# lasgroup/safe-adaptation-gym

Measured on AMD Instinct MI355X. Metric: env-steps/sec (batched) Point/GoToGoal, higher is better.
Workload: dtype f32

## Files before the change

safe_adaptation_gym_amd/csrc/sag_device.hpp:

```cpp
#pragma once
#include <hip/hip_runtime.h>
#include <stdint.h>

#include <type_traits>

#include "../../include/sag.h"

namespace sag {

constexpr int WAVE = 64;

enum { DI_META = 0, DI_TSTATE = 1, DI_STEP = 2, DI_ENVID = 3, DI_FLAGS = 4, DI_COUNT = 5 };
constexpr int FLAG_EPISODE_SHIFT = 8;
__host__ __device__ constexpr size_t ipad(size_t N) { return (N + 3) & ~(size_t)3; }
__host__ __device__ constexpr size_t icount(size_t N) { return ipad(N) + 4 * N; }
__host__ __device__ constexpr size_t iaddr(int w, size_t N, size_t i) {
  return w == DI_TSTATE ? i : ipad(N) + i * 4 + (w == DI_META ? 0 : (w == DI_STEP ? 1 : (w == DI_ENVID ? 2 : 3)));
}

constexpr int DEV_FLOATS = 192, DEV_GROUPS = DEV_FLOATS / 4;
constexpr int DV_POS = 40, DV_VEL = 76, DG_HAZ = 5, DG_POS = 10, DG_PILLARS = 4, DG_BUTTONS = 28;
__host__ __device__ constexpr int didx(int k) {
  return k < 6 ? k
       : k < 9 ? 136 + (k - 6)
       : k < 12 ? k
       : k < 14 ? k
       : k < 24 ? 140 + (k - 14)
       : k == 24 ? 38
       : k < 27 ? 14 + (k - 25)
       : k < 32 ? 130 + (k - 27)
       : k < 34 ? 6 + (k - 32)
       : k < 38 ? 124 + (k - 34)
       : k == 38 ? 8
       : k < 41 ? 128 + (k - 39)
       : k < 44 ? DV_POS + 30 + (k - 41)
       : k < 47 ? DV_VEL + 30 + (k - 44)
       : k < 65 ? 20 + (k - 47)
       : k < 69 ? 16 + (k - 65)
       : k < 81 ? 112 + (k - 69)
       : k < 141 ? ((k - 81) % 6 < 3 ? DV_POS + 3 * ((k - 81) / 6) + (k - 81) % 6
                                     : DV_VEL + 3 * ((k - 81) / 6) + (k - 81) % 6 - 3)
       : k == 141 ? 39
       : k < 144 ? 150 + (k - 142)
       : 152 + (k - 144);
}
static_assert(didx(SAG_F_BUTTONS) == 112 && didx(SAG_F_VASES + 6 * 3 + 4) == DV_VEL + 10 && didx(SAG_F_BOX + 1) == DV_POS + 31 &&
              didx(SAG_F_HAZARDS) == 4 * DG_HAZ && didx(SAG_F_PILLARS) == 4 * DG_PILLARS, "device layout constants");
__host__ __device__ constexpr size_t saddr(int k, size_t N, size_t i) {
  return ((size_t)(didx(k) >> 2) * N + i) * 4 + (didx(k) & 3);
}

__host__ __device__ inline uint32_t pack_meta(const int32_t* ri) {
  return (uint32_t)ri[SAG_I_TASK] | (uint32_t)ri[SAG_I_NH] << 4 | (uint32_t)ri[SAG_I_NV] << 8 |
         (uint32_t)ri[SAG_I_NP] << 12 | (uint32_t)ri[SAG_I_NB] << 14 |
         (uint32_t)ri[SAG_I_BOX_KIND] << 17;
}
__host__ __device__ inline void unpack_meta(uint32_t m, int32_t* ri) {
  ri[SAG_I_TASK] = m & 15; ri[SAG_I_NH] = m >> 4 & 15; ri[SAG_I_NV] = m >> 8 & 15;
  ri[SAG_I_NP] = m >> 12 & 3; ri[SAG_I_NB] = m >> 14 & 7; ri[SAG_I_BOX_KIND] = m >> 17 & 3;
}
__host__ __device__ inline uint32_t pack_tstate(const int32_t* ri) {
  return (uint32_t)ri[SAG_I_GOAL_BUTTON] | (uint32_t)ri[SAG_I_BTN_STATE] << 3 |
         (uint32_t)ri[SAG_I_BTN_TIMER] << 4 | (uint32_t)ri[SAG_I_CATCH_TIMER] << 7 |
         (uint32_t)ri[SAG_I_ACTIVE_MASK] << 11;
}
__host__ __device__ inline void unpack_tstate(uint32_t t, int32_t* ri) {
  ri[SAG_I_GOAL_BUTTON] = t & 7; ri[SAG_I_BTN_STATE] = t >> 3 & 1; ri[SAG_I_BTN_TIMER] = t >> 4 & 7;
  ri[SAG_I_CATCH_TIMER] = t >> 7 & 15; ri[SAG_I_ACTIVE_MASK] = t >> 11 & 63;
}

// ... 755 lines not shown
  auto G4 = [&](int g) { return S4[(size_t)g * N + i]; };
  const bool use_hot = MODE == MODE_BUSY && p.hot != nullptr;
  const float4* __restrict__ H4 = use_hot ? reinterpret_cast<const float4*>(p.hot) + (size_t)i * HOT_GROUPS : nullptr;
  auto GH = [&](int g, int hslot) { return use_hot ? H4[hslot] : G4(g); };
  int4 iw;
  uint32_t tstate;
  if (use_hot) {
    const float4 hi = H4[14], ht = H4[15];
    iw = make_int4(__float_as_int(hi.x), __float_as_int(hi.y), __float_as_int(hi.z), __float_as_int(hi.w));
    tstate = (uint32_t)__float_as_int(ht.x);
  } else {
    iw = reinterpret_cast<const int4*>(I + ipad((size_t)N))[i];
    tstate = (uint32_t)I[iaddr(DI_TSTATE, (size_t)N, (size_t)i)];
  }
  const uint32_t meta = (uint32_t)iw.x;
  int step = iw.y;
  const uint32_t env_id = (uint32_t)iw.z;
  const float4 gA = GH(0, 0), gB = GH(1, 1), gC = GH(2, 2), gD = GH(3, 3);
  BV R;
  R.x = gA.x; R.y = gA.y;
  float yaw = gA.z;
  R.vx = gA.w; R.vy = gB.x; R.w = gB.y;
  R.ax = R.ay = R.aw = 0; R.dyn = 1;
  const float gear = gC.y, damp = gC.z;
  const float vsz = gD.z, psz = gD.w;
  float ext[9] = {0, 0, 0, 0, 0, 1, 0, 0, 0}, eacc[5] = {0, 0, 0, 0, 0};
  constexpr int DG_EXT = (152 >> 2);
  static_assert(didx(SAG_F_ROBOT_EXT) == 152 && didx(SAG_F_ROBOT_EXT + 8) == 160, "car extension = device groups 38..40");
  float4 ext_tail = make_float4(0.f, 0.f, 0.f, 0.f);
  if constexpr (CAR) {
    const float4 e0 = G4(DG_EXT), e1 = G4(DG_EXT + 1);
    ext_tail = G4(DG_EXT + 2);
    ext[0] = e0.x; ext[1] = e0.y; ext[2] = e0.z; ext[3] = e0.w; ext[4] = e1.x; ext[5] = e1.y; ext[6] = e1.z; ext[7] = e1.w;
    ext[8] = ext_tail.x;
    if constexpr (PARK) {
      CPK(CP_Q) = ext[5]; CPK(CP_Q + 1) = ext[6]; CPK(CP_Q + 2) = ext[7]; CPK(CP_Q + 3) = ext[8];
      CPK(CP_TAIL) = ext_tail.y; CPK(CP_TAIL + 1) = ext_tail.z; CPK(CP_TAIL + 2) = ext_tail.w;
    }
  }
  float goalx = gB.z, goaly = gB.w;
  float last0 = gC.x;
  float a0 = 0, a1 = 0, n0 = 0, n1 = 0;
  if (!p.observe_only) {
    if constexpr (!DOGGO) {
      const float2 a = reinterpret_cast<const float2*>(p.actions)[i];
      a0 = a.x; a1 = a.y;
      if (p.noise) { const float2 z = reinterpret_cast<const float2*>(p.noise)[i]; n0 = z.x; n1 = z.y; }
    }
  }
  {
    float vpos[36];
    const int need = HAS_TBOX && p.has_box ? 9 : (3 * capV + 3) / 4;
#pragma unroll
    for (int g = 0; g < 9; g++) {
      float4 v = make_float4(0.f, 0.f, 0.f, 0.f);
      if (g < need) v = GH(DG_POS + g, 5 + g);
      vpos[4 * g] = v.x; vpos[4 * g + 1] = v.y; vpos[4 * g + 2] = v.z; vpos[4 * g + 3] = v.w;
    }
#pragma unroll
    for (int k = 0; k < SAG_MAX_VASES; k++)
      if (k >= capV) { vpos[3 * k] = vpos[3 * k + 1] = vpos[3 * k + 2] = 0; }
    if (!(HAS_TBOX && p.has_box)) { vpos[3 * BOX_ID] = vpos[3 * BOX_ID + 1] = vpos[3 * BOX_ID + 2] = 0; }
#pragma unroll
    for (int k = 0; k < NBODY; k++) { LP(LS_X, k) = vpos[3 * k]; LP(LS_Y, k) = vpos[3 * k + 1]; LP(LS_YAW, k) = vpos[3 * k + 2]; }
  }
  float stx[NSTAT], sty[NSTAT];
  {
    float4 v = make_float4(0.f, 0.f, 0.f, 0.f);
    if (capP > 0) v = GH(DG_PILLARS, 4);
    stx[0] = v.x; sty[0] = v.y; stx[1] = capP > 1 ? v.z : 0.f; sty[1] = capP > 1 ? v.w : 0.f;
    static_assert(SAG_MAX_PILLARS == 2, "pillars fill one group");
  }
  if constexpr (HAS_BTN) {
    float bt[12];
#pragma unroll
    for (int g = 0; g < 3; g++) {
      float4 v = make_float4(0.f, 0.f, 0.f, 0.f);
      if (2 * g < capB) v = G4(DG_BUTTONS + g);
      bt[4 * g] = v.x; bt[4 * g + 1] = v.y; bt[4 * g + 2] = v.z; bt[4 * g + 3] = v.w;
    }
    static_assert(SAG_MAX_BUTTONS == 6, "buttons fill three groups");
#pragma unroll
    for (int k = 0; k < SAG_MAX_BUTTONS; k++) {
      stx[SAG_MAX_PILLARS + k] = k < capB ? bt[2 * k] : 0.f;
      sty[SAG_MAX_PILLARS + k] = k < capB ? bt[2 * k + 1] : 0.f;
    }
  }
// ... 15 lines not shown
    if (!p.observe_only) {
      const float an = SF(SAG_F_ACTION_NOISE);
#pragma unroll 1
      for (int j = 0; j < 12; j += 2) {
        float z0, z1;
        if (p.noise) { z0 = p.noise[(size_t)i * 12 + j]; z1 = p.noise[(size_t)i * 12 + j + 1]; }
        else {
          uint32_t c[4] = {rng.env, rng.step, (uint32_t)(j >> 1), rng.ep4 | 1u};
          philox4x32_10(c, p.key0, p.key1);
          box_muller(c[0], c[1], z0, z1);
        }
        const float l0 = SF(SAG_F_CTRL_SCALE + j), l1 = SF(SAG_F_CTRL_SCALE + j + 1);
        ctrl12[j] = clampf(p.actions[(size_t)i * 12 + j] + an * z0, -l0, l0);
        ctrl12[j + 1] = clampf(p.actions[(size_t)i * 12 + j + 1] + an * z1, -l1, l1);
      }
    }
  }
  if (!p.observe_only) {
    if (!p.noise && !DOGGO) {
      uint32_t c[4] = {rng.env, rng.step, 0u, rng.ep4 | 1u};
      philox4x32_10(c, p.key0, p.key1);
      box_muller(c[0], c[1], n0, n1);
    }
    const float an = gC.w;
    const float cs0 = gD.x, cs1 = gD.y;
    ctrl0 = clampf(a0 + an * n0, -cs0, cs0);
    ctrl1 = clampf(a1 + an * n1, -cs1, cs1);
    if (task == SAG_TASK_CATCH_GOAL) {
      int t = tstate >> 7 & 15;
      t = t - 1 > 0 ? t - 1 : 0;
      float cur = SF(SAG_F_CATCH + 2), nxt = SF(SAG_F_CATCH + 3);
      if (t == 0) {
        cur = nxt;
        nxt = (float)rng.uniform(0.2, 1.0);
        if (rng.exhausted) flags |= 2;
        if (live) { SF(SAG_F_CATCH + 2) = cur; SF(SAG_F_CATCH + 3) = nxt; }
        t = 10;
      }
      tstate = (tstate & ~(15u << 7)) | (uint32_t)t << 7;
      double time = (double)step * p.nstep_table * (double)p.h;
      double progress = (10 - t) / 10.0;
      double radius = progress * ((double)nxt - (double)cur) + (double)cur;
      goalx = (float)((double)SF(SAG_F_CATCH) + sin(time) * radius);
      goaly = (float)((double)SF(SAG_F_CATCH + 1) + cos(time) * radius);
    }
  }

  const float h = p.h;
// ... 86 lines not shown
      dgr.cost_contacts = (int)dr[15]; dgr.btn_mask = (uint32_t)dr[16]; dgr.overflow = (int)dr[17];
    } else {
      static_assert(post, "the Doggo physics is k_doggo_physics (sag_doggo_coop.hpp); the generic step only post-processes its results");
    }
    cost_contacts = dgr.cost_contacts; btn_mask = dgr.btn_mask;
    if (dgr.overflow) flags |= 4;
    float wz;
    if (!p.observe_only && live && !post) dg_store(dgs, S, (size_t)N, (size_t)i, yaw, wz);
    else { double Rm[9], ww[3]; dg_quat2mat(dgs.quat, Rm); dg_matvec(Rm, dgs.wloc, ww); yaw = (float)atan2(Rm[3], Rm[0]); wz = (float)ww[2]; }
    {
      double Rm[9];
      dg_quat2mat(dgs.quat, Rm);
      for (int k = 0; k < 9; k++) dg_rot[k] = Rm[k];
    }
    R.x = (float)dgs.pos[0]; R.y = (float)dgs.pos[1]; R.vx = (float)dgs.vlin[0]; R.vy = (float)dgs.vlin[1]; R.w = wz;
    R.ax = (float)dgr.qacc_lin[0]; R.ay = (float)dgr.qacc_lin[1];
    if (nsub > 0) awake = 0;
    for (int k = 0; k < NBODY; k++) {
      const bool isb = k == BOX_ID;
      if (isb ? !has_box : k >= nV) continue;
      LP(LS_X, k) = Wd.fb[k][0]; LP(LS_Y, k) = Wd.fb[k][1]; LP(LS_YAW, k) = Wd.fb[k][2];
      if (Wd.fb[k][3] != 0 || Wd.fb[k][4] != 0 || Wd.fb[k][5] != 0) awake |= 1u << k;
      if (!p.observe_only && live && !post) {
        for (int c = 0; c < 3; c++) { SD(DV_POS + 3 * k + c) = Wd.fb[k][c]; SD(DV_VEL + 3 * k + c) = Wd.fb[k][3 + c]; }
      }
    }
  } else {
  float car_f0 = 0, car_f1 = 0, car_f2 = 0, car_px = 0, car_py = 0, car_pw = 0;
  float car_fL = 0, car_fT = 0, car_fR = 0, car_fX = 0, car_fY = 0;
  bool car_warm = false;
  auto car_floor = [&](const float a0, const float a1, const float a2) {
#pragma clang fp contract(on)
    constexpr float CM = CAR_M, CIO = CAR_IO, COY = CAR_OY, CJD = 0.001f, CRW = 0.05f, AB = -CM * COY;
    constexpr float CNL = CM * GRAV * (0.1f + COY) / 0.4f, CNC = CM * GRAV - 2 * CNL;
    constexpr float IDC = 1.0f / (CM * (CM * CIO - AB * AB));
    constexpr float M0 = (CM * CIO) * IDC, M2 = (-AB * CM) * IDC, M3 = (CM * CIO - AB * AB) * IDC, M5 = (CM * CM) * IDC;
    constexpr float UL0 = -0.13f * M2, UL2 = -0.13f * M5, UT0 = M0 - 0.1f * M2, UT2 = M2 - 0.1f * M5, UX0 = M0 + 0.1f * M2, UX2 = M2 + 0.1f * M5;
    constexpr float LIML = MU * CNL, LIMT = 2 * MU * CNL, LIMC = MU * CNC;
    const float vbx = cy * R.vx + sy * R.vy, vby = cy * R.vy - sy * R.vx, bc = sol0.bcoef;
    const float qL = (clampf(ctrl0, -0.02f, 0.02f) - CJD * ext[0]) * p.car.iIw, qR = (clampf(ctrl1, -0.02f, 0.02f) - CJD * ext[1]) * p.car.iIw;
    const float qX = CJD * ext[3] * p.car.iIb, qY = -CJD * ext[2] * p.car.iIb;
    const float rL = -bc * (vby - 0.13f * R.w + CRW * ext[0]), rT = -bc * (vbx - 0.1f * R.w), rR = -bc * (vby + 0.13f * R.w + CRW * ext[1]);
    const float rX = -bc * (vbx + 0.1f * R.w - CRW * ext[3]), rY = -bc * (vby + CRW * ext[2]);
    const float cL = rL - CRW * qL, cR = rR - CRW * qR, cX = rX - CRW * qX, cY = rY - CRW * qY;
    float fL, fT, fR, fX, fY;
    if constexpr (PARK) { fL = CPK(CP_FL); fT = CPK(CP_FL + 1); fR = CPK(CP_FL + 2); fX = CPK(CP_FL + 3); fY = CPK(CP_FL + 4); }
    else { fL = car_fL; fT = car_fT; fR = car_fR; fX = car_fX; fY = car_fY; }
// ... 332 lines not shown
    ext_tail.y = CPK(CP_TAIL); ext_tail.z = CPK(CP_TAIL + 1); ext_tail.w = CPK(CP_TAIL + 2);
  }

  }
  if (p.ext_cc) {
    const int32_t v = p.ext_cc[i];
    if (v >= 0) { cost_contacts = v; btn_mask = p.ext_btn[i]; }
  }
  CYC(CY_ROBOT);
  const float boxx = LP(LS_X, BOX_ID), boxy = LP(LS_Y, BOX_ID);
  if (!p.observe_only && live) {
    if constexpr (!DOGGO) {
      float4* __restrict__ W4 = reinterpret_cast<float4*>(S);
      W4[(size_t)0 * N + i] = make_float4(R.x, R.y, yaw, R.vx);
    }
    if constexpr (CAR) {
      float4* __restrict__ W4 = reinterpret_cast<float4*>(S);
      W4[(size_t)DG_EXT * N + i] = make_float4(ext[0], ext[1], ext[2], ext[3]);
      W4[(size_t)(DG_EXT + 1) * N + i] = make_float4(ext[4], ext[5], ext[6], ext[7]);
      W4[(size_t)(DG_EXT + 2) * N + i] = make_float4(ext[8], ext_tail.y, ext_tail.z, ext_tail.w);
    }
    for (uint32_t m = dirty; m; m &= m - 1) {
      const int k = __ffs(m) - 1;
      const int f = DV_POS + 3 * k, fv = DV_VEL + 3 * k;
      SD(f) = LP(LS_X, k); SD(f + 1) = LP(LS_Y, k); SD(f + 2) = LP(LS_YAW, k);
      const int d = dy.slot(k);
      if (d >= 0) { SD(fv) = POOL(d, 0); SD(fv + 1) = POOL(d, 1); SD(fv + 2) = POOL(d, 2); }
    }
    step += 1;
    reinterpret_cast<int4*>(I + ipad((size_t)N))[i] = make_int4(iw.x, step, iw.z, iw.w);
  }
  tstate = (tstate & ~(TS_AWAKE_BITS << TS_AWAKE_SHIFT)) | (awake & TS_AWAKE_BITS) << TS_AWAKE_SHIFT;
  bool busy_next = false;
  if (!p.observe_only) {
    const float T = p.nstep_table * h;
    const float amax = CAR ? GRAV : 1.05f * gear * PT_FLIM / PT_MASS;
    const float reach = sqrtf(R.vx * R.vx + R.vy * R.vy) * T + amax * T * T + 0.005f;
    bool busy = awake != 0 || (HAS_TBOX && task == SAG_TASK_HAUL_BOX);
    bool near_obj = false, near_static = false;
    const bool moving = busy;
    const float rr = my_bound + reach;
    constexpr bool FINE = !CAR && !DOGGO;
    const float dth = (fmaxf(fabsf(R.w), 3.0f) + 1.0f) * T;
    const float fa = 0.1f + reach, fb = 0.0707107f + reach + 0.1f * dth;
    const float Bx = R.x + 0.1f * cy, By = R.y + 0.1f * sy;
#pragma unroll 1
    for (int k = 0; k < nV; k++) {
      const float vx_ = LP(LS_X, k), vy_ = LP(LS_Y, k);
      const float dx = vx_ - R.x, dyy = vy_ - R.y, rs = rr + vase_r;
      if (dx * dx + dyy * dyy <= rs * rs) {
        if constexpr (FINE) {
          float sv, cv; sincosf(LP(LS_YAW, k), &sv, &cv);
          auto box_d2 = [&](float px, float py) {
            const float wx = px - vx_, wy = py - vy_;
            const float ex = fmaxf(fabsf(cv * wx + sv * wy) - vsz, 0.f), ey = fmaxf(fabsf(cv * wy - sv * wx) - vsz, 0.f);
            return ex * ex + ey * ey;
          };
          busy |= box_d2(R.x, R.y) <= fa * fa || box_d2(Bx, By) <= fb * fb;
        } else busy = true;
      }
    }
    if (has_box) {
      const float dx = LP(LS_X, BOX_ID) - R.x, dyy = LP(LS_Y, BOX_ID) - R.y, rs = rr + box_r;
      near_obj = dx * dx + dyy * dyy <= rs * rs;
    }
#pragma unroll 1
    for (int k = 0; k < n_static; k++) {
      if (k == capP) k = SAG_MAX_PILLARS;
      const bool is_p = k < SAG_MAX_PILLARS;
      const bool on = is_p ? (k < nP) : (k - SAG_MAX_PILLARS < nB);
      const float sr = is_p ? psz : BUTTON_R;
      const float skx = pick(stx, k), sky = pick(sty, k);
      const float dx = skx - R.x, dyy = sky - R.y, rs = rr + sr;
      if constexpr (FINE) {
        const float ex = skx - Bx, ey = sky - By;
        near_static |= on && (dx * dx + dyy * dyy <= (fa + sr) * (fa + sr) || ex * ex + ey * ey <= (fb + sr) * (fb + sr));
      } else near_static |= on && dx * dx + dyy * dyy <= rs * rs;
    }
    const bool near_vase = busy && !moving;
    busy |= near_obj || near_static;
    const uint32_t kind = p.busy_kinds ? (uint32_t)near_obj | (uint32_t)near_static << 1 | (uint32_t)(near_vase || moving) << 2 : 0u;
    const uint32_t nbit = TS_BUSY_BIT << (p.phase ^ 1);
    tstate = busy ? (tstate | nbit) : (tstate & ~nbit);
    if (busy && live && p.kind) p.kind[i] = (uint8_t)kind;
    busy_next = busy;
  }

  CYC(CY_WRITEBACK);
  float hzx[SAG_MAX_HAZARDS], hzy[SAG_MAX_HAZARDS];
  float hsz;
  {
    float hz[20];
#pragma unroll
    for (int g = 0; g < 5; g++) {
      float4 v = make_float4(0.f, 0.f, 0.f, 0.f);
      if (g == 4 || 2 * g < capH) v = use_hot ? reinterpret_cast<const float4*>(p.hot_haz)[(size_t)i * 5 + g] : G4(DG_HAZ + g);
      hz[4 * g] = v.x; hz[4 * g + 1] = v.y; hz[4 * g + 2] = v.z; hz[4 * g + 3] = v.w;
    }
    static_assert(SAG_MAX_HAZARDS == 9, "hazards + size fill five groups");
#pragma unroll
    for (int k = 0; k < SAG_MAX_HAZARDS; k++) { hzx[k] = k < capH ? hz[2 * k] : 0.f; hzy[k] = k < capH ? hz[2 * k + 1] : 0.f; }
    hsz = hz[18];
  }

  bool bad = false;
  {
    float v[6] = {R.x, R.y, yaw, R.vx, R.vy, R.w};
#pragma unroll
    for (int k = 0; k < 6; k++) bad |= !(fabsf(v[k]) <= 1e10f);
    if constexpr (DOGGO) {
      bad |= !(fabs(dgs.pos[2]) <= 1e10) || !(fabs(dgs.vlin[2]) <= 1e10);
      for (int k = 0; k < 4; k++) bad |= !(fabs(dgs.quat[k]) <= 1e10);
      for (int k = 0; k < 3; k++) bad |= !(fabs(dgs.wloc[k]) <= 1e10);
      for (int k = 0; k < DG_NJ; k++) bad |= !(fabs(dgs.q[k]) <= 1e10) || !(fabs(dgs.qd[k]) <= 1e10);
    }
  }

  double rew0 = 0, rew1 = 0;
  int met = 0;
  const double rx = R.x, ry = R.y;
  bool need_goal = false;
  float box_last1 = 0, box_last2 = 0;
  if (!p.observe_only && !bad) {
    if (task == SAG_TASK_PRESS_BUTTONS || task == SAG_TASK_PRESS_BUTTONS_SCARCE) {
      int gb = tstate & 7, bstate = tstate >> 3 & 1, timer = tstate >> 4 & 7;
// ... 143 lines not shown
    }
  }
  CYC(CY_RESAMPLE);
  if (!p.observe_only && !bad) {
    if (need_goal) {
      last0 = (float)dist2d(rx, ry, goalx, goaly);
      if (task == SAG_TASK_CATCH_GOAL && live) { SF(SAG_F_CATCH) = goalx; SF(SAG_F_CATCH + 1) = goaly; }
      if (has_box) {
        box_last2 = (float)dist2d(goalx, goaly, boxx, boxy);
        box_last1 = (float)dist2d(rx, ry, boxx, boxy);
      }
    }
    if (live) {
      if (has_box) { SF(SAG_F_LAST + 1) = box_last1; SF(SAG_F_LAST + 2) = box_last2; }
      if constexpr (DOGGO) {
        SF(SAG_F_LAST) = last0;
        SF(SAG_F_GOAL) = goalx; SF(SAG_F_GOAL + 1) = goaly;
      }
    }
  }
  if constexpr (!DOGGO) {
    if (!p.observe_only && live) {
      float4* __restrict__ W4 = reinterpret_cast<float4*>(S);
      W4[(size_t)1 * N + i] = make_float4(R.vy, R.w, bad ? gB.z : goalx, bad ? gB.w : goaly);
      W4[(size_t)2 * N + i] = make_float4(bad ? gC.x : last0, gC.y, gC.z, gC.w);
    }
  }
  if (!p.observe_only && live) I[iaddr(DI_TSTATE, (size_t)N, (size_t)i)] = (int32_t)tstate;
  if constexpr (MODE != MODE_ALL && !DOGGO) {
    if (p.hot && busy_next && live && !p.observe_only) {
      float4* __restrict__ Hw = reinterpret_cast<float4*>(p.hot) + (size_t)i * HOT_GROUPS;
      Hw[0] = make_float4(R.x, R.y, yaw, R.vx);
      Hw[1] = make_float4(R.vy, R.w, bad ? gB.z : goalx, bad ? gB.w : goaly);
      Hw[2] = make_float4(bad ? gC.x : last0, gC.y, gC.z, gC.w);
      Hw[3] = gD;
      Hw[4] = make_float4(stx[0], sty[0], stx[1], sty[1]);
#pragma unroll
      for (int g = 0; g < 9; g++) {
        float v[4];
#pragma unroll
        for (int c = 0; c < 4; c++) {
          const int f = 4 * g + c, k = f / 3, comp = f % 3;
          v[c] = k < NBODY ? lds[((comp == 0 ? LS_X : (comp == 1 ? LS_Y : LS_YAW)) + k) * WAVE + lane] : 0.f;
        }
        Hw[5 + g] = make_float4(v[0], v[1], v[2], v[3]);
      }
      Hw[14] = make_float4(__int_as_float(iw.x), __int_as_float(step), __int_as_float(iw.z), __int_as_float(iw.w | flags));
      Hw[15] = make_float4(__int_as_float((int)tstate), 0.f, 0.f, 0.f);
    }
  }

  int cost = 0;
  if (!p.observe_only && !bad) {
    int c = cost_contacts;
#pragma unroll 1
    for (int k = 0; k < SAG_MAX_HAZARDS; k++) {
      if (k < nH) {
        const float dx = R.x - hzx[k], dyy = R.y - hzy[k];
        const float d2 = dx * dx + dyy * dyy, t2 = hsz * hsz;
        bool in = d2 <= t2;
        if (fabsf(d2 - t2) < 1e-5f) in = dist2d(rx, ry, hzx[k], hzy[k]) <= (double)hsz;
        c += in;
      }
    }
    cost = c > 0;
  }
// ... 230 lines not shown
  const bool live = gi < p.N && lane < epw;
  step_body<ROBOT, HAS_BTN, HAS_TBOX, MODE_ALL>(p, lds, lane, live ? gi : p.N - 1, live, base,
                                                 min(epw, p.N - base), 0ull, nullptr);
}

template <bool HAS_BTN, bool HAS_TBOX>
__global__ __launch_bounds__(WAVE, 1) void k_step_doggo_post(StepArgs p) {
  __shared__ float lds[LDS_FLOATS];
  const int lane = threadIdx.x, base = blockIdx.x * WAVE, gi = base + lane;
  const bool live = gi < p.N;
  step_body<SAG_ROBOT_DOGGO, HAS_BTN, HAS_TBOX, MODE_POST>(p, lds, lane, live ? gi : p.N - 1, live, base, min(WAVE, p.N - base),
                                                            0ull, nullptr);
}

#ifndef SAG_QUIET_MIN_WAVES
#define SAG_QUIET_MIN_WAVES 4
#endif
#ifndef SAG_CAR_QUIET_MIN_WAVES
#define SAG_CAR_QUIET_MIN_WAVES 3
#endif
template <int ROBOT, bool HAS_BTN, bool HAS_TBOX>
__global__ __launch_bounds__(WAVE, ROBOT == SAG_ROBOT_CAR ? SAG_CAR_QUIET_MIN_WAVES : SAG_QUIET_MIN_WAVES) void k_step_quiet(StepArgs p) {
  constexpr int QSLOTS = quiet_lds_rows(ROBOT, HAS_BTN, HAS_TBOX);
  static_assert(QSLOTS >= LS_YAW + NBODY, "the yaw rows written at load time must stay in bounds");
  static_assert(QSLOTS * WAVE * (int)sizeof(float) <= quiet_lds_total(ROBOT), "the quiet array stays inside the footprint of its launch");
  __shared__ float lds[QSLOTS * WAVE];
  const int lane = threadIdx.x, base = blockIdx.x * WAVE, gi = base + lane;
  const bool in = gi < p.N;
  const bool busy = in && ((uint32_t)p.I[iaddr(DI_TSTATE, (size_t)p.N, (size_t)gi)] & (TS_BUSY_BIT << p.phase));
  const uint64_t skip = __ballot(busy || !in);
  if (skip == ~0ull) return;
  const bool live = in && !busy;
  step_body<ROBOT, HAS_BTN, HAS_TBOX, MODE_QUIET>(p, lds, lane, in ? gi : p.N - 1, live, base,
                                                   min(WAVE, p.N - base), skip, nullptr);
}

constexpr int COMPACT_PER_LANE = 16, COMPACT_ENVS = 256 * COMPACT_PER_LANE;
template <bool KINDS>
__global__ __launch_bounds__(256) void k_compact(const int32_t* I, const uint8_t* kind, int N, int phase, int32_t* rows, int32_t* count,
                                                  int32_t* zero_for_next, const int32_t* prev_total, int kinds_min) {
  constexpr int NC = KINDS ? BUSY_CLASSES : 1;
  const bool use_kinds = KINDS && *prev_total > kinds_min;
  if (blockIdx.x == 0 && threadIdx.x < BUSY_CLASSES) zero_for_next[threadIdx.x] = 0;
  __shared__ int wave_tot[4][BUSY_CLASSES];
  __shared__ int wave_base[4][BUSY_CLASSES];
  const int lane = threadIdx.x & 63, wv = threadIdx.x >> 6;
  const int e0 = blockIdx.x * COMPACT_ENVS + wv * (WAVE * COMPACT_PER_LANE);
// ... 59 lines not shown
#pragma unroll
  for (int k = 0; k < BUSY_CLASSES; k++) {
    const int c = busy_class_order(k), n = p.count[c], w = (n + WAVE - 1) / WAVE;
    if (cls < 0) { if (b < w) { cls = c; count = n; } else b -= w; }
  }
  if (cls < 0) return;
  const int lane = threadIdx.x, c0 = b * WAVE;
  const int nval = min(WAVE, count - c0);
  const bool live = lane < nval;
  const int i = p.rows[(size_t)cls * p.N + c0 + (live ? lane : 0)];
  rows[lane] = i;
  __syncthreads();
  step_body<ROBOT, HAS_BTN, HAS_TBOX, MODE_BUSY>(p, lds, lane, i, live, 0, nval, 0ull, rows);
#ifdef SAG_WAVE_TIMES
  if (lane == 0 && blockIdx.x < WT_MAX) { g_wt[blockIdx.x][0] = wt0; g_wt[blockIdx.x][1] = wall_clock64(); }
#endif
}

__device__ inline void hot_refresh_env(const float* __restrict__ S, const int32_t* __restrict__ I, int N, size_t i,
                                       float* __restrict__ hot, float* __restrict__ hot_haz) {
  const float4* S4 = reinterpret_cast<const float4*>(S);
  float4* H = reinterpret_cast<float4*>(hot) + i * HOT_GROUPS;
  for (int g = 0; g < 5; g++) H[g] = S4[(size_t)g * N + i];
  for (int g = 0; g < 9; g++) H[5 + g] = S4[(size_t)(DG_POS + g) * N + i];
  const int4 iw = reinterpret_cast<const int4*>(I + ipad((size_t)N))[i];
  H[14] = make_float4(__int_as_float(iw.x), __int_as_float(iw.y), __int_as_float(iw.z), __int_as_float(iw.w));
  H[15] = make_float4(__int_as_float(I[i]), 0.f, 0.f, 0.f);
  float4* Z = reinterpret_cast<float4*>(hot_haz) + i * 5;
  for (int g = 0; g < 5; g++) Z[g] = S4[(size_t)(DG_HAZ + g) * N + i];
}

__global__ __launch_bounds__(256) void k_hot_refresh(const float* __restrict__ S, const int32_t* __restrict__ I, int N,
                                                      float* __restrict__ hot, float* __restrict__ hot_haz) {
  const size_t i = (size_t)blockIdx.x * blockDim.x + threadIdx.x;
  if (i < (size_t)N) hot_refresh_env(S, I, N, i, hot, hot_haz);
}

__device__ inline void install_env(float* S, int32_t* I, int N, int i, const float* rf, const int32_t* ri, int init_task) {
  for (int k = 0; k < SAG_REC_FLOATS; k++) S[saddr(k, (size_t)N, (size_t)i)] = rf[k];
  uint32_t awake = init_task ? 0u : (uint32_t)ri[SAG_I_AWAKE] & TS_AWAKE_BITS;
  {
    const int nV = ri[SAG_I_NV], bkind = ri[SAG_I_BOX_KIND], nP = ri[SAG_I_NP], nB = ri[SAG_I_NB];
    const float vsz = rf[SAG_F_VASE_SIZE], psz = rf[SAG_F_PILLAR_SIZE];
    auto exists = [&](int a) { return a < SAG_MAX_VASES ? a < nV : bkind != SAG_BOX_NONE; };
    auto rec = [&](int a) { return a < SAG_MAX_VASES ? rf + SAG_F_VASES + 6 * a : rf + SAG_F_BOX; };
    auto bound = [&](int a) {
      return a < SAG_MAX_VASES ? shape_bound(SH_VASE, vsz, 0.f)
// ... 418 lines not shown
```

safe_adaptation_gym_amd/csrc/sag_doggo_coop.hpp:

```cpp
#pragma once

namespace sag {

constexpr int DC_ROWS = DG_MAXROWS;
constexpr int DC_PGS_LANES = 32;
#ifndef SAG_DC_FAST_ROWS
#define SAG_DC_FAST_ROWS DC_PGS_LANES
#endif
struct DcContact {
  double dir[3][3], c[3], depth;
  float bcoef, kcoef, mu;
  uint32_t key;
  short body, other;
  short touch, dbl;
};
struct DcEnv {
  double pos[3], quat[4], q[DG_NJ], vlin[3], wloc[3], qd[DG_NJ];
  union {
    struct {
      double R[DG_NB][9], p[DG_NB][3];
      double S[DG_NV][6];
      double Ib[DG_NB][10];
      union {
        struct {
// ... 901 lines not shown
    W.vk.reff = vsz * 1.41421356237309504880f;
    W.bk.sh = SH_BOX; W.bk.m = 1; W.bk.I = 1; W.bk.reff = 0.2f * 1.41421356237309504880f;
    if (box_kind == SAG_BOX_BOX) {
      const float m0 = 0.001f * 0.064f, m1 = 0.001f * 0.016f;
      W.bk.m = m0 + 4 * m1; W.bk.I = m0 * 0.32f / 12 + 4 * (m1 * 0.08f / 12 + m1 * 0.08f);
    } else if (box_kind == SAG_BOX_ROD) {
      W.bk.sh = SH_ROD; W.bk.m = 0.0005f * (3.14159265358979323846f * 0.08f * 0.08f * 0.6f);
      W.bk.I = W.bk.m * (3 * 0.08f * 0.08f + 0.36f) / 12;
    } else if (box_kind == SAG_BOX_BALL) {
      W.bk.sh = SH_BALL; W.bk.m = 0.0005f * (4.0f / 3.0f * 3.14159265358979323846f * 0.14f * 0.14f * 0.14f);
      W.bk.I = 0.4f * W.bk.m * 0.14f * 0.14f;
    }
  }
  const float vase_r = W.vk.reff, box_r = shape_bound(W.bk.sh, W.vsz, 0);
  const double top_vase = 2.0 * (double)W.vsz;
  const double top_box = W.bk.sh == SH_ROD ? 0.16 : (W.bk.sh == SH_BALL ? 0.28 : 0.4);

  dc_load_model();
  dc_load_state(hf, u, S, N, i);
  if (u < NBODY) {
    const int k = u;
    const bool isb = k == BOX_ID, on = isb ? W.has_box : k < W.nV;
    for (int c = 0; c < 3; c++) {
      E.wfb[k][c] = on ? S[((size_t)((DV_POS + 3 * k + c) >> 2) * N + i) * 4 + ((DV_POS + 3 * k + c) & 3)] : 0.f;
      E.wfb[k][3 + c] = on ? S[((size_t)((DV_VEL + 3 * k + c) >> 2) * N + i) * 4 + ((DV_VEL + 3 * k + c) & 3)] : 0.f;
      E.wfb[k][6 + c] = 0.f;
    }
    for (int c = 0; c < 6; c++) E.wminv[k][c] = 0;
    if (!isb) { E.wminv[k][0] = E.wminv[k][3] = 1.0f / W.vk.m; E.wminv[k][5] = 1.0f / W.vk.I; }
    else {
      E.wminv[k][5] = 1.0f / W.bk.I;
      E.wminv[k][0] = E.wminv[k][3] = W.bk.sh == SH_BALL ? 1.0f / (1.4f * W.bk.m) : 1.0f / W.bk.m;
    }
  }
  if (u < SAG_MAX_PILLARS + SAG_MAX_BUTTONS) {
    const int f = u < SAG_MAX_PILLARS ? SAG_F_PILLARS + 2 * u : SAG_F_BUTTONS + 2 * (u - SAG_MAX_PILLARS);
    stx_s[half][u] = S[saddr(f, N, i)]; sty_s[half][u] = S[saddr(f + 1, N, i)];
  }
  if (u < 12) {
    float c = 0;
    if (!p.observe_only) {
      float z;
      if (p.noise) z = p.noise[i * 12 + u];
      else {
        const uint32_t env_id = (uint32_t)p.I[iaddr(DI_ENVID, N, i)], step = (uint32_t)p.I[iaddr(DI_STEP, N, i)];
        const uint32_t ep4 = ((uint32_t)p.I[iaddr(DI_FLAGS, N, i)] >> FLAG_EPISODE_SHIFT) << 2;
        uint32_t cc[4] = {env_id, step, (uint32_t)(u >> 1), ep4 | 1u};
// ... 313 lines not shown
    sc[16 + ((size_t)((p.dg_phase + 1) & 1) * DC_NCLS + cls) * N + slot] = (int32_t)gi;
  }
  if (live) {
    double* dr = DR + gi * DR_STRIDE;
    if (u < 3) dr[u] = E.qacc[u];
    if (u < 8) dr[3 + u] = E.touch[u];
    if (u == 0) {
      dr[11] = E.com[0]; dr[12] = E.com[1]; dr[13] = E.mom[0]; dr[14] = E.mom[1];
      dr[15] = (double)cost_contacts; dr[16] = (double)btn_mask; dr[17] = (E.flag & 2) ? 1.0 : 0.0;
    }
    if (!p.observe_only) {
      if (u == 0) {
        DgState D;
        for (int k = 0; k < 3; k++) { D.pos[k] = E.pos[k]; D.vlin[k] = E.vlin[k]; D.wloc[k] = E.wloc[k]; }
        for (int k = 0; k < 4; k++) D.quat[k] = E.quat[k];
        for (int j = 0; j < DG_NJ; j++) { D.q[j] = E.q[j]; D.qd[j] = E.qd[j]; }
        float yaw, wz;
        dg_store(D, S, N, gi, yaw, wz);
      }
      if (u < NBODY) {
        const bool isb = u == BOX_ID;
        if (isb ? W.has_box : u < W.nV)
          for (int c = 0; c < 3; c++) {
            S[((size_t)((DV_POS + 3 * u + c) >> 2) * N + gi) * 4 + ((DV_POS + 3 * u + c) & 3)] = E.wfb[u][c];
            S[((size_t)((DV_VEL + 3 * u + c) >> 2) * N + gi) * 4 + ((DV_VEL + 3 * u + c) & 3)] = E.wfb[u][3 + c];
          }
      }
    }
  }
#ifdef SAG_CYCLES
  DCC(DCY_STORE);
  if (lane == 0) {
    unsigned long long tot = 0;
    for (int k = 0; k < DCY_N; k++) { atomicAdd(&g_cyc[1][k], g_dc_cyc[k]); tot += g_dc_cyc[k]; }
    atomicAdd(&g_cyc[1][CY_N], 1ull);
    atomicAdd(&g_cyc[2][min((int)(tot >> 19), CY_N)], 1ull);
  }
#endif
}

}
```

Baseline: 4.549 billion.

## Split free-body pose into xy and yaw runs and defer yaw loads in quiet path

Reorders the device state layout so free-body (x, y) and yaw live in separate contiguous runs. The robot scalar groups are also reshuffled so goal and last-action fields sit together. In the quiet kernel, yaw groups are fetched only for lanes whose circle test finds a nearby vase, object or static. Group 2 of the state is written back only when the goal can change. This targets global memory traffic per step, at the cost of a more intricate layout and a second, deferred load phase.

```diff
diff --git a/safe_adaptation_gym_amd/csrc/sag_device.hpp b/safe_adaptation_gym_amd/csrc/sag_device.hpp
--- a/safe_adaptation_gym_amd/csrc/sag_device.hpp
+++ b/safe_adaptation_gym_amd/csrc/sag_device.hpp
@@ -19,33 +19,50 @@
 }
 
 constexpr int DEV_FLOATS = 192, DEV_GROUPS = DEV_FLOATS / 4;
-constexpr int DV_POS = 40, DV_VEL = 76, DG_HAZ = 5, DG_POS = 10, DG_PILLARS = 4, DG_BUTTONS = 28;
+constexpr int DV_XY = 40, DV_YAW = 64, DV_VEL = 76, DG_HAZ = 5, DG_XY = DV_XY / 4, DG_YAW = DV_YAW / 4, DG_PILLARS = 4, DG_BUTTONS = 28;
+constexpr int XY_GROUPS = 6, YAW_GROUPS = 3;
 __host__ __device__ constexpr int didx(int k) {
   return k < 6 ? k
        : k < 9 ? 136 + (k - 6)
-       : k < 12 ? k
-       : k < 14 ? k
+       : k < 11 ? 10 + (k - 9)
+       : k < 14 ? 12 + (k - 11)
        : k < 24 ? 140 + (k - 14)
        : k == 24 ? 38
-       : k < 27 ? 14 + (k - 25)
+       : k == 25 ? 15
+       : k == 26 ? 7
        : k < 32 ? 130 + (k - 27)
-       : k < 34 ? 6 + (k - 32)
+       : k < 34 ? 8 + (k - 32)
        : k < 38 ? 124 + (k - 34)
-       : k == 38 ? 8
+       : k == 38 ? 6
        : k < 41 ? 128 + (k - 39)
-       : k < 44 ? DV_POS + 30 + (k - 41)
+       : k < 43 ? DV_XY + 2 * SAG_MAX_VASES + (k - 41)
+       : k == 43 ? DV_YAW + SAG_MAX_VASES
        : k < 47 ? DV_VEL + 30 + (k - 44)
        : k < 65 ? 20 + (k - 47)
        : k < 69 ? 16 + (k - 65)
        : k < 81 ? 112 + (k - 69)
-       : k < 141 ? ((k - 81) % 6 < 3 ? DV_POS + 3 * ((k - 81) / 6) + (k - 81) % 6
-                                     : DV_VEL + 3 * ((k - 81) / 6) + (k - 81) % 6 - 3)
+       : k < 141 ? ((k - 81) % 6 < 2 ? DV_XY + 2 * ((k - 81) / 6) + (k - 81) % 6
+                    : (k - 81) % 6 == 2 ? DV_YAW + (k - 81) / 6
+                                        : DV_VEL + 3 * ((k - 81) / 6) + (k - 81) % 6 - 3)
        : k == 141 ? 39
        : k < 144 ? 150 + (k - 142)
        : 152 + (k - 144);
 }
-static_assert(didx(SAG_F_BUTTONS) == 112 && didx(SAG_F_VASES + 6 * 3 + 4) == DV_VEL + 10 && didx(SAG_F_BOX + 1) == DV_POS + 31 &&
+static_assert(didx(SAG_F_BUTTONS) == 112 && didx(SAG_F_VASES + 6 * 3 + 4) == DV_VEL + 10 && didx(SAG_F_BOX + 1) == DV_XY + 21 &&
               didx(SAG_F_HAZARDS) == 4 * DG_HAZ && didx(SAG_F_PILLARS) == 4 * DG_PILLARS, "device layout constants");
+static_assert(didx(SAG_F_VASES) == DV_XY && didx(SAG_F_VASES + 6 * 9 + 1) == DV_XY + 19 && didx(SAG_F_BOX) == DV_XY + 2 * SAG_MAX_VASES &&
+              didx(SAG_F_VASES + 2) == DV_YAW && didx(SAG_F_VASES + 6 * 9 + 2) == DV_YAW + 9 && didx(SAG_F_BOX + 2) == DV_YAW + SAG_MAX_VASES &&
+              DV_XY + 4 * XY_GROUPS == DV_YAW && DV_YAW + 4 * YAW_GROUPS == DV_VEL, "the (x, y) run and the yaw run of the free bodies");
+constexpr bool didx_is_a_layout() {
+  bool used[DEV_FLOATS] = {};
+  for (int k = 0; k < SAG_REC_FLOATS; k++) {
+    const int d = didx(k);
+    if (d < 0 || d >= DEV_FLOATS || used[d]) return false;
+    used[d] = true;
+  }
+  return true;
+}
+static_assert(didx_is_a_layout(), "didx is injective over the record floats and stays below DEV_FLOATS");
 __host__ __device__ constexpr size_t saddr(int k, size_t N, size_t i) {
   return ((size_t)(didx(k) >> 2) * N + i) * 4 + (didx(k) & 3);
 }
@@ -847,8 +864,8 @@
   float yaw = gA.z;
   R.vx = gA.w; R.vy = gB.x; R.w = gB.y;
   R.ax = R.ay = R.aw = 0; R.dyn = 1;
-  const float gear = gC.y, damp = gC.z;
-  const float vsz = gD.z, psz = gD.w;
+  const float gear = gC.z, damp = gC.w;
+  const float vsz = gD.w, psz = gB.w;
   float ext[9] = {0, 0, 0, 0, 0, 1, 0, 0, 0}, eacc[5] = {0, 0, 0, 0, 0};
   constexpr int DG_EXT = (152 >> 2);
   static_assert(didx(SAG_F_ROBOT_EXT) == 152 && didx(SAG_F_ROBOT_EXT + 8) == 160, "car extension = device groups 38..40");
@@ -863,8 +880,8 @@
       CPK(CP_TAIL) = ext_tail.y; CPK(CP_TAIL + 1) = ext_tail.z; CPK(CP_TAIL + 2) = ext_tail.w;
     }
   }
-  float goalx = gB.z, goaly = gB.w;
-  float last0 = gC.x;
+  float goalx = gC.x, goaly = gC.y;
+  float last0 = gB.z;
   float a0 = 0, a1 = 0, n0 = 0, n1 = 0;
   if (!p.observe_only) {
     if constexpr (!DOGGO) {
@@ -873,21 +890,42 @@
       if (p.noise) { const float2 z = reinterpret_cast<const float2*>(p.noise)[i]; n0 = z.x; n1 = z.y; }
     }
   }
+  const bool box_ctx = HAS_TBOX && p.has_box;
+  const int need_xy = box_ctx ? XY_GROUPS : (2 * capV + 3) / 4, need_yaw = box_ctx ? YAW_GROUPS : (capV + 3) / 4;
   {
-    float vpos[36];
-    const int need = HAS_TBOX && p.has_box ? 9 : (3 * capV + 3) / 4;
-#pragma unroll
-    for (int g = 0; g < 9; g++) {
+    float vxy[4 * XY_GROUPS];
+#pragma unroll
+    for (int g = 0; g < XY_GROUPS; g++) {
       float4 v = make_float4(0.f, 0.f, 0.f, 0.f);
-      if (g < need) v = GH(DG_POS + g, 5 + g);
-      vpos[4 * g] = v.x; vpos[4 * g + 1] = v.y; vpos[4 * g + 2] = v.z; vpos[4 * g + 3] = v.w;
+      if (g < need_xy) v = GH(DG_XY + g, 5 + g);
+      vxy[4 * g] = v.x; vxy[4 * g + 1] = v.y; vxy[4 * g + 2] = v.z; vxy[4 * g + 3] = v.w;
     }
 #pragma unroll
     for (int k = 0; k < SAG_MAX_VASES; k++)
-      if (k >= capV) { vpos[3 * k] = vpos[3 * k + 1] = vpos[3 * k + 2] = 0; }
-    if (!(HAS_TBOX && p.has_box)) { vpos[3 * BOX_ID] = vpos[3 * BOX_ID + 1] = vpos[3 * BOX_ID + 2] = 0; }
-#pragma unroll
-    for (int k = 0; k < NBODY; k++) { LP(LS_X, k) = vpos[3 * k]; LP(LS_Y, k) = vpos[3 * k + 1]; LP(LS_YAW, k) = vpos[3 * k + 2]; }
+      if (k >= capV) { vxy[2 * k] = vxy[2 * k + 1] = 0; }
+    if (!box_ctx) { vxy[2 * BOX_ID] = vxy[2 * BOX_ID + 1] = 0; }
+#pragma unroll
+    for (int k = 0; k < NBODY; k++) { LP(LS_X, k) = vxy[2 * k]; LP(LS_Y, k) = vxy[2 * k + 1]; }
+  }
+  auto put_yaw = [&](const float4 (&yg)[YAW_GROUPS]) {
+    float vy_[4 * YAW_GROUPS];
+#pragma unroll
+    for (int g = 0; g < YAW_GROUPS; g++) { vy_[4 * g] = yg[g].x; vy_[4 * g + 1] = yg[g].y; vy_[4 * g + 2] = yg[g].z; vy_[4 * g + 3] = yg[g].w; }
+#pragma unroll
+    for (int k = 0; k < SAG_MAX_VASES; k++)
+      if (k >= capV) vy_[k] = 0;
+    if (!box_ctx) vy_[BOX_ID] = 0;
+#pragma unroll
+    for (int k = 0; k < NBODY; k++) LP(LS_YAW, k) = vy_[k];
+  };
+  if constexpr (!QUIET) {
+    float4 yg[YAW_GROUPS];
+#pragma unroll
+    for (int g = 0; g < YAW_GROUPS; g++) {
+      yg[g] = make_float4(0.f, 0.f, 0.f, 0.f);
+      if (g < need_yaw) yg[g] = GH(DG_YAW + g, 5 + XY_GROUPS + g);
+    }
+    put_yaw(yg);
   }
   float stx[NSTAT], sty[NSTAT];
   {
@@ -949,8 +987,8 @@
       philox4x32_10(c, p.key0, p.key1);
       box_muller(c[0], c[1], n0, n1);
     }
-    const float an = gC.w;
-    const float cs0 = gD.x, cs1 = gD.y;
+    const float an = gD.x;
+    const float cs0 = gD.y, cs1 = gD.z;
     ctrl0 = clampf(a0 + an * n0, -cs0, cs0);
     ctrl1 = clampf(a1 + an * n1, -cs1, cs1);
     if (task == SAG_TASK_CATCH_GOAL) {
@@ -1083,7 +1121,8 @@
       LP(LS_X, k) = Wd.fb[k][0]; LP(LS_Y, k) = Wd.fb[k][1]; LP(LS_YAW, k) = Wd.fb[k][2];
       if (Wd.fb[k][3] != 0 || Wd.fb[k][4] != 0 || Wd.fb[k][5] != 0) awake |= 1u << k;
       if (!p.observe_only && live && !post) {
-        for (int c = 0; c < 3; c++) { SD(DV_POS + 3 * k + c) = Wd.fb[k][c]; SD(DV_VEL + 3 * k + c) = Wd.fb[k][3 + c]; }
+        SD(DV_XY + 2 * k) = Wd.fb[k][0]; SD(DV_XY + 2 * k + 1) = Wd.fb[k][1]; SD(DV_YAW + k) = Wd.fb[k][2];
+        for (int c = 0; c < 3; c++) SD(DV_VEL + 3 * k + c) = Wd.fb[k][3 + c];
       }
     }
   } else {
@@ -1462,8 +1501,8 @@
     }
     for (uint32_t m = dirty; m; m &= m - 1) {
       const int k = __ffs(m) - 1;
-      const int f = DV_POS + 3 * k, fv = DV_VEL + 3 * k;
-      SD(f) = LP(LS_X, k); SD(f + 1) = LP(LS_Y, k); SD(f + 2) = LP(LS_YAW, k);
+      const int f = DV_XY + 2 * k, fv = DV_VEL + 3 * k;
+      SD(f) = LP(LS_X, k); SD(f + 1) = LP(LS_Y, k); SD(DV_YAW + k) = LP(LS_YAW, k);
       const int d = dy.slot(k);
       if (d >= 0) { SD(fv) = POOL(d, 0); SD(fv + 1) = POOL(d, 1); SD(fv + 2) = POOL(d, 2); }
     }
@@ -1472,38 +1511,31 @@
   }
   tstate = (tstate & ~(TS_AWAKE_BITS << TS_AWAKE_SHIFT)) | (awake & TS_AWAKE_BITS) << TS_AWAKE_SHIFT;
   bool busy_next = false;
-  if (!p.observe_only) {
-    const float T = p.nstep_table * h;
-    const float amax = CAR ? GRAV : 1.05f * gear * PT_FLIM / PT_MASS;
-    const float reach = sqrtf(R.vx * R.vx + R.vy * R.vy) * T + amax * T * T + 0.005f;
-    bool busy = awake != 0 || (HAS_TBOX && task == SAG_TASK_HAUL_BOX);
-    bool near_obj = false, near_static = false;
-    const bool moving = busy;
-    const float rr = my_bound + reach;
-    constexpr bool FINE = !CAR && !DOGGO;
-    const float dth = (fmaxf(fabsf(R.w), 3.0f) + 1.0f) * T;
-    const float fa = 0.1f + reach, fb = 0.0707107f + reach + 0.1f * dth;
-    const float Bx = R.x + 0.1f * cy, By = R.y + 0.1f * sy;
-#pragma unroll 1
-    for (int k = 0; k < nV; k++) {
-      const float vx_ = LP(LS_X, k), vy_ = LP(LS_Y, k);
-      const float dx = vx_ - R.x, dyy = vy_ - R.y, rs = rr + vase_r;
-      if (dx * dx + dyy * dyy <= rs * rs) {
-        if constexpr (FINE) {
-          float sv, cv; sincosf(LP(LS_YAW, k), &sv, &cv);
-          auto box_d2 = [&](float px, float py) {
-            const float wx = px - vx_, wy = py - vy_;
-            const float ex = fmaxf(fabsf(cv * wx + sv * wy) - vsz, 0.f), ey = fmaxf(fabsf(cv * wy - sv * wx) - vsz, 0.f);
-            return ex * ex + ey * ey;
-          };
-          busy |= box_d2(R.x, R.y) <= fa * fa || box_d2(Bx, By) <= fb * fb;
-        } else busy = true;
-      }
-    }
-    if (has_box) {
-      const float dx = LP(LS_X, BOX_ID) - R.x, dyy = LP(LS_Y, BOX_ID) - R.y, rs = rr + box_r;
-      near_obj = dx * dx + dyy * dyy <= rs * rs;
-    }
+  const float T = p.nstep_table * h;
+  const float amax = CAR ? GRAV : 1.05f * gear * PT_FLIM / PT_MASS;
+  const float reach = sqrtf(R.vx * R.vx + R.vy * R.vy) * T + amax * T * T + 0.005f;
+  const bool moving = awake != 0 || (HAS_TBOX && task == SAG_TASK_HAUL_BOX);
+  const float rr = my_bound + reach;
+  constexpr bool FINE = !CAR && !DOGGO;
+  const float dth = (fmaxf(fabsf(R.w), 3.0f) + 1.0f) * T;
+  const float fa = 0.1f + reach, fb = 0.0707107f + reach + 0.1f * dth;
+  const float Bx = R.x + 0.1f * cy, By = R.y + 0.1f * sy;
+  auto vase_fine = [&](int k, float vx_, float vy_) {
+    float sv, cv; sincosf(LP(LS_YAW, k), &sv, &cv);
+    auto box_d2 = [&](float px, float py) {
+      const float wx = px - vx_, wy = py - vy_;
+      const float ex = fmaxf(fabsf(cv * wx + sv * wy) - vsz, 0.f), ey = fmaxf(fabsf(cv * wy - sv * wx) - vsz, 0.f);
+      return ex * ex + ey * ey;
+    };
+    return box_d2(R.x, R.y) <= fa * fa || box_d2(Bx, By) <= fb * fb;
+  };
+  auto object_near = [&]() {
+    if (!has_box) return false;
+    const float dx = LP(LS_X, BOX_ID) - R.x, dyy = LP(LS_Y, BOX_ID) - R.y, rs = rr + box_r;
+    return dx * dx + dyy * dyy <= rs * rs;
+  };
+  auto static_near = [&]() {
+    bool near_static = false;
 #pragma unroll 1
     for (int k = 0; k < n_static; k++) {
       if (k == capP) k = SAG_MAX_PILLARS;
@@ -1517,13 +1549,52 @@
         near_static |= on && (dx * dx + dyy * dyy <= (fa + sr) * (fa + sr) || ex * ex + ey * ey <= (fb + sr) * (fb + sr));
       } else near_static |= on && dx * dx + dyy * dyy <= rs * rs;
     }
-    const bool near_vase = busy && !moving;
-    busy |= near_obj || near_static;
+    return near_static;
+  };
+  auto classified = [&](bool near_vase, bool near_obj, bool near_static) {
+    const bool busy = moving || near_vase || near_obj || near_static;
     const uint32_t kind = p.busy_kinds ? (uint32_t)near_obj | (uint32_t)near_static << 1 | (uint32_t)(near_vase || moving) << 2 : 0u;
     const uint32_t nbit = TS_BUSY_BIT << (p.phase ^ 1);
     tstate = busy ? (tstate | nbit) : (tstate & ~nbit);
     if (busy && live && p.kind) p.kind[i] = (uint8_t)kind;
     busy_next = busy;
+  };
+  if constexpr (!QUIET) {
+    if (!p.observe_only) {
+      bool near_vase = false;
+#pragma unroll 1
+      for (int k = 0; k < nV; k++) {
+        const float vx_ = LP(LS_X, k), vy_ = LP(LS_Y, k);
+        const float dx = vx_ - R.x, dyy = vy_ - R.y, rs = rr + vase_r;
+        if (dx * dx + dyy * dyy <= rs * rs) {
+          if constexpr (FINE) near_vase |= vase_fine(k, vx_, vy_);
+          else near_vase = true;
+        }
+      }
+      const bool near_obj = object_near(), near_static = static_near();
+      classified(near_vase, near_obj, near_static);
+    }
+  }
+  uint32_t circ_v = 0;
+  bool q_obj = false, q_static = false, q_cand = false;
+  float4 q_yaw[YAW_GROUPS];
+#pragma unroll
+  for (int g = 0; g < YAW_GROUPS; g++) q_yaw[g] = make_float4(0.f, 0.f, 0.f, 0.f);
+  if constexpr (QUIET) {
+    if (!p.observe_only) {
+#pragma unroll 1
+      for (int k = 0; k < nV; k++) {
+        const float dx = LP(LS_X, k) - R.x, dyy = LP(LS_Y, k) - R.y, rs = rr + vase_r;
+        if (dx * dx + dyy * dyy <= rs * rs) circ_v |= 1u << k;
+      }
+      q_obj = object_near(); q_static = static_near();
+      q_cand = live && (circ_v != 0 || q_obj || q_static || moving);
+      if (q_cand) {
+#pragma unroll
+        for (int g = 0; g < YAW_GROUPS; g++)
+          if (g < need_yaw) q_yaw[g] = G4(DG_YAW + g);
+      }
+    }
   }
 
   CYC(CY_WRITEBACK);
@@ -1541,6 +1612,21 @@
 #pragma unroll
     for (int k = 0; k < SAG_MAX_HAZARDS; k++) { hzx[k] = k < capH ? hz[2 * k] : 0.f; hzy[k] = k < capH ? hz[2 * k + 1] : 0.f; }
     hsz = hz[18];
+  }
+  if constexpr (QUIET) {
+    if (!p.observe_only) {
+      bool near_vase = false;
+      if (q_cand) {
+        put_yaw(q_yaw);
+        if constexpr (FINE) {
+          for (uint32_t m = circ_v; m; m &= m - 1) {
+            const int k = __ffs(m) - 1;
+            near_vase |= vase_fine(k, LP(LS_X, k), LP(LS_Y, k));
+          }
+        } else near_vase = circ_v != 0;
+      }
+      classified(near_vase, q_obj, q_static);
+    }
   }
 
   bool bad = false;
@@ -1730,8 +1816,8 @@
   if constexpr (!DOGGO) {
     if (!p.observe_only && live) {
       float4* __restrict__ W4 = reinterpret_cast<float4*>(S);
-      W4[(size_t)1 * N + i] = make_float4(R.vy, R.w, bad ? gB.z : goalx, bad ? gB.w : goaly);
-      W4[(size_t)2 * N + i] = make_float4(bad ? gC.x : last0, gC.y, gC.z, gC.w);
+      W4[(size_t)1 * N + i] = make_float4(R.vy, R.w, bad ? gB.z : last0, gB.w);
+      if (!bad && (need_goal || task == SAG_TASK_CATCH_GOAL)) W4[(size_t)2 * N + i] = make_float4(goalx, goaly, gC.z, gC.w);
     }
   }
   if (!p.observe_only && live) I[iaddr(DI_TSTATE, (size_t)N, (size_t)i)] = (int32_t)tstate;
@@ -1739,17 +1825,17 @@
     if (p.hot && busy_next && live && !p.observe_only) {
       float4* __restrict__ Hw = reinterpret_cast<float4*>(p.hot) + (size_t)i * HOT_GROUPS;
       Hw[0] = make_float4(R.x, R.y, yaw, R.vx);
-      Hw[1] = make_float4(R.vy, R.w, bad ? gB.z : goalx, bad ? gB.w : goaly);
-      Hw[2] = make_float4(bad ? gC.x : last0, gC.y, gC.z, gC.w);
+      Hw[1] = make_float4(R.vy, R.w, bad ? gB.z : last0, gB.w);
+      Hw[2] = make_float4(bad ? gC.x : goalx, bad ? gC.y : goaly, gC.z, gC.w);
       Hw[3] = gD;
       Hw[4] = make_float4(stx[0], sty[0], stx[1], sty[1]);
 #pragma unroll
-      for (int g = 0; g < 9; g++) {
+      for (int g = 0; g < XY_GROUPS + YAW_GROUPS; g++) {
         float v[4];
 #pragma unroll
         for (int c = 0; c < 4; c++) {
-          const int f = 4 * g + c, k = f / 3, comp = f % 3;
-          v[c] = k < NBODY ? lds[((comp == 0 ? LS_X : (comp == 1 ? LS_Y : LS_YAW)) + k) * WAVE + lane] : 0.f;
+          const int f = 4 * (g < XY_GROUPS ? g : g - XY_GROUPS) + c, k = g < XY_GROUPS ? f / 2 : f;
+          v[c] = k < NBODY ? lds[((g < XY_GROUPS ? (f % 2 == 0 ? LS_X : LS_Y) : LS_YAW) + k) * WAVE + lane] : 0.f;
         }
         Hw[5 + g] = make_float4(v[0], v[1], v[2], v[3]);
       }
@@ -2026,7 +2112,7 @@
 template <int ROBOT, bool HAS_BTN, bool HAS_TBOX>
 __global__ __launch_bounds__(WAVE, ROBOT == SAG_ROBOT_CAR ? SAG_CAR_QUIET_MIN_WAVES : SAG_QUIET_MIN_WAVES) void k_step_quiet(StepArgs p) {
   constexpr int QSLOTS = quiet_lds_rows(ROBOT, HAS_BTN, HAS_TBOX);
-  static_assert(QSLOTS >= LS_YAW + NBODY, "the yaw rows written at load time must stay in bounds");
+  static_assert(QSLOTS >= LS_YAW + NBODY, "the yaw rows a lane within reach of something writes (classification) must stay in bounds");
   static_assert(QSLOTS * WAVE * (int)sizeof(float) <= quiet_lds_total(ROBOT), "the quiet array stays inside the footprint of its launch");
   __shared__ float lds[QSLOTS * WAVE];
   const int lane = threadIdx.x, base = blockIdx.x * WAVE, gi = base + lane;
@@ -2132,7 +2218,7 @@
   const float4* S4 = reinterpret_cast<const float4*>(S);
   float4* H = reinterpret_cast<float4*>(hot) + i * HOT_GROUPS;
   for (int g = 0; g < 5; g++) H[g] = S4[(size_t)g * N + i];
-  for (int g = 0; g < 9; g++) H[5 + g] = S4[(size_t)(DG_POS + g) * N + i];
+  for (int g = 0; g < XY_GROUPS + YAW_GROUPS; g++) H[5 + g] = S4[(size_t)(DG_XY + g) * N + i];
   const int4 iw = reinterpret_cast<const int4*>(I + ipad((size_t)N))[i];
   H[14] = make_float4(__int_as_float(iw.x), __int_as_float(iw.y), __int_as_float(iw.z), __int_as_float(iw.w));
   H[15] = make_float4(__int_as_float(I[i]), 0.f, 0.f, 0.f);
diff --git a/safe_adaptation_gym_amd/csrc/sag_doggo_coop.hpp b/safe_adaptation_gym_amd/csrc/sag_doggo_coop.hpp
--- a/safe_adaptation_gym_amd/csrc/sag_doggo_coop.hpp
+++ b/safe_adaptation_gym_amd/csrc/sag_doggo_coop.hpp
@@ -947,7 +947,8 @@
     const int k = u;
     const bool isb = k == BOX_ID, on = isb ? W.has_box : k < W.nV;
     for (int c = 0; c < 3; c++) {
-      E.wfb[k][c] = on ? S[((size_t)((DV_POS + 3 * k + c) >> 2) * N + i) * 4 + ((DV_POS + 3 * k + c) & 3)] : 0.f;
+      const int dp = c < 2 ? DV_XY + 2 * k + c : DV_YAW + k;
+      E.wfb[k][c] = on ? S[((size_t)(dp >> 2) * N + i) * 4 + (dp & 3)] : 0.f;
       E.wfb[k][3 + c] = on ? S[((size_t)((DV_VEL + 3 * k + c) >> 2) * N + i) * 4 + ((DV_VEL + 3 * k + c) & 3)] : 0.f;
       E.wfb[k][6 + c] = 0.f;
     }
@@ -1307,7 +1308,8 @@
         const bool isb = u == BOX_ID;
         if (isb ? W.has_box : u < W.nV)
           for (int c = 0; c < 3; c++) {
-            S[((size_t)((DV_POS + 3 * u + c) >> 2) * N + gi) * 4 + ((DV_POS + 3 * u + c) & 3)] = E.wfb[u][c];
+            const int dp = c < 2 ? DV_XY + 2 * u + c : DV_YAW + u;
+            S[((size_t)(dp >> 2) * N + gi) * 4 + (dp & 3)] = E.wfb[u][c];
             S[((size_t)((DV_VEL + 3 * u + c) >> 2) * N + gi) * 4 + ((DV_VEL + 3 * u + c) & 3)] = E.wfb[u][3 + c];
           }
       }
```

Measured after the change: 4.799 billion, median of 6. 1.05x the previous value.
